# AnishDelft/ModelCompression

Measured on AMD Instinct MI355X. Metric: images/sec (fwd+bwd, 416x416), higher is better.
Workload: dtype fp16

## Files before the change

include/mcamd.h:

```cpp
#ifndef MCAMD_H
#define MCAMD_H

#include <stddef.h>
#include <stdint.h>

#ifdef __cplusplus
extern "C" {
#endif

#define MCAMD_OK 0
#define MCAMD_EINVAL (-1)
#define MCAMD_ELAUNCH (-2)
#define MCAMD_EWORKSPACE (-3)

int mcamd_version(void);
void mcamd_reload_config(void);
const char* mcamd_arch(void);
const char* mcamd_last_error(void);

typedef struct mcamd_conv_geom {
    int32_t B, H, W;
    int32_t ksize;
    int32_t cin;
    int32_t cout;
    int32_t x_ld;
    int32_t x_choff;
    int32_t stem;
    int32_t pad;
    int32_t x_wrap;
    int32_t x_f8;
    int32_t x_f8_wexp;
} mcamd_conv_geom;
int32_t mcamd_conv_fwd_f8_ok(const mcamd_conv_geom* g);

#define MCAMD_EPI_RAW_F16 0
#define MCAMD_EPI_NCHW_F32 1
#define MCAMD_EPI_PAD_F16 2
#define MCAMD_EPI_RAW_F32 3
typedef struct mcamd_conv_epilogue {
    int32_t mode;
    int32_t y_ld, y_choff;
    void* y;
    const float* bias;
    float* stats;
    int32_t stats_rows;
    int32_t stats_ld;
    const float* scale;
    const float* shift;
    float slope;
    int32_t* overflow;
    int32_t dst_mode;
    void* y2;
    int32_t y2_ld, y2_choff;
    int32_t concurrent;
} mcamd_conv_epilogue;

int32_t mcamd_conv_stats_rows(const mcamd_conv_geom* g);
int32_t mcamd_conv_stats_rows_mode(const mcamd_conv_geom* g, int32_t mode);

int mcamd_conv_tile_info(const mcamd_conv_geom* g, int32_t dgrad, int32_t out[4]);
int mcamd_conv_route_info(const mcamd_conv_geom* g, int32_t dir, int32_t mode, int32_t dst_mode, int32_t stats, int32_t out[5]);

int64_t mcamd_packed_elems_fwd(const mcamd_conv_geom* g);
int64_t mcamd_packed_elems_dgrad(const mcamd_conv_geom* g);

typedef struct mcamd_chan_map {
    const int32_t* rows;
    const int32_t* cols;
} mcamd_chan_map;

int mcamd_pack_weights(const mcamd_conv_geom* g, const float* w_oihw, const float* mask_oihw,
                       const mcamd_chan_map* map, void* wp_fwd, void* wp_dgrad, void* stream);

typedef struct mcamd_pack_job {
    const float* w;
    const float* mask;
    void* dst_fwd;
    void* dst_dgrad;
    const int32_t* rows;
    const int32_t* cols;
    int64_t first_tile;
    int32_t cout, cin, ksize;
    int32_t split;
    int32_t f8_wexp;
} mcamd_pack_job;
int mcamd_pack_weights_many(const mcamd_pack_job* jobs_dev, int32_t njobs, int64_t total_tiles, void* stream);

int mcamd_conv_fwd(const mcamd_conv_geom* g, const void* x, const void* wp_fwd,
                   const mcamd_conv_epilogue* epi, void* stream);

int32_t mcamd_conv_fwd_sparse24_ok(const mcamd_conv_geom* g);
int mcamd_sparse24_elems(const mcamd_conv_geom* g, int64_t out[2]);
int mcamd_conv_fwd_sparse24_info(const mcamd_conv_geom* g, int32_t out[7]);
int mcamd_pack_sparse24(const mcamd_conv_geom* g, const float* w_oihw, const float* mask_oihw, void* wsp, void* idx, void* stream);
int mcamd_conv_fwd_sparse24(const mcamd_conv_geom* g, const void* x, const void* wsp, const void* idx,
                            const mcamd_conv_epilogue* epi, void* stream);

int32_t mcamd_conv_fwd_bsparse_ok(const mcamd_conv_geom* g);
int mcamd_bsparse_elems(const mcamd_conv_geom* g, int64_t out[2]);
int mcamd_bsparse_lists(const mcamd_conv_geom* g, const void* wp_fwd, int32_t* count, int32_t* list, void* stream);
int mcamd_conv_fwd_bsparse(const mcamd_conv_geom* g, const void* x, const void* wp_fwd, const int32_t* count,
                           const int32_t* list, const mcamd_conv_epilogue* epi, void* stream);

typedef struct mcamd_splitk_info {
    int32_t slices;
    int32_t bm, bn, bk;
    int32_t chunks;
    int32_t tiles;
    int64_t workspace_bytes;
} mcamd_splitk_info;
int mcamd_conv_fwd_splitk_info(const mcamd_conv_geom* g, int32_t mode, int32_t dst_mode, int32_t slices,
                               mcamd_splitk_info* out);
int mcamd_conv_fwd_splitk(const mcamd_conv_geom* g, const void* x, const void* wp_fwd, const mcamd_conv_epilogue* epi,
                          int32_t slices, void* workspace, size_t workspace_bytes, void* stream);

int32_t mcamd_conv_fwd_q8_ok(const mcamd_conv_geom* g);
int mcamd_q8_elems(const mcamd_conv_geom* g, int64_t out[2]);
int mcamd_pack_q8(const mcamd_conv_geom* g, const float* w_oihw, const float* mask_oihw, void* wq, int32_t* wexp, void* stream);
int mcamd_conv_fwd_q8(const mcamd_conv_geom* g, const void* x8, const void* wq, const int32_t* wexp,
                      const mcamd_conv_epilogue* epi, int32_t y_f8, int32_t y2_f8, void* stream);
int mcamd_conv_fwd_q8_info(const mcamd_conv_geom* g, int32_t form, int32_t out[7]);
int mcamd_cast_q8(const void* src, int64_t pixels, int32_t src_ld, int32_t src_choff, int32_t C, void* dst, int32_t dst_ld,
                  int32_t dst_choff, void* stream);

int mcamd_conv_fwd_q8_splitk_info(const mcamd_conv_geom* g, int32_t dst_mode, int32_t slices, mcamd_splitk_info* out);
int mcamd_conv_fwd_q8_splitk(const mcamd_conv_geom* g, const void* x8, const void* wq, const int32_t* wexp,
                             const mcamd_conv_epilogue* epi, int32_t y_f8, int32_t y2_f8, int32_t slices, void* workspace,
                             size_t workspace_bytes, void* stream);

int32_t mcamd_conv_fwd_q8_slim_ok(const mcamd_conv_geom* g);
int mcamd_q8_slim_elems(const mcamd_conv_geom* g, int64_t out[2]);
int mcamd_pack_q8_slim(const mcamd_conv_geom* g, const float* w_oihw, const float* mask_oihw, void* wq, int32_t* wexp,
                       void* stream);
int mcamd_conv_fwd_q8_slim(const mcamd_conv_geom* g, const void* x8, const void* wq, const int32_t* wexp,
                           const mcamd_conv_epilogue* epi, const float* border, int32_t border_ld, int32_t y_f8, int32_t y2_f8,
                           void* stream);

int32_t mcamd_conv_fwd_q8_stats_rows(const mcamd_conv_geom* g);
int mcamd_fakequant_q8(const mcamd_conv_geom* g, const float* w_oihw, const float* mask_oihw, const int32_t* wexp,
                       float* wq_oihw, void* stream);
int mcamd_cast_q8_train(void* src, int64_t pixels, int32_t src_ld, int32_t src_choff, int32_t C, void* dst, int32_t dst_ld,
                        int32_t dst_choff, void* stream);

int32_t mcamd_conv_fwd_q8_sparse24_ok(const mcamd_conv_geom* g);
int mcamd_q8_sparse24_elems(const mcamd_conv_geom* g, int64_t out[3]);
int mcamd_pack_q8_sparse24(const mcamd_conv_geom* g, const float* w_oihw, const float* mask_oihw, void* wq, void* idx,
                           int32_t* wexp, void* stream);
int mcamd_conv_fwd_q8_sparse24(const mcamd_conv_geom* g, const void* x8, const void* wq, const void* idx, const int32_t* wexp,
                               const mcamd_conv_epilogue* epi, int32_t y_f8, int32_t y2_f8, void* stream);

int32_t mcamd_conv_fwd_q8_w4_ok(const mcamd_conv_geom* g);
int mcamd_q8_w4_elems(const mcamd_conv_geom* g, int64_t out[3]);
int mcamd_pack_q8_w4(const mcamd_conv_geom* g, const float* w_oihw, const float* mask_oihw, void* codes, void* gshift,
                     int32_t* wexp, void* stream);
int mcamd_unpack_q8_w4(const mcamd_conv_geom* g, const void* codes, const void* gshift, void* wq, void* stream);
int mcamd_conv_fwd_q8_w4(const mcamd_conv_geom* g, const void* x8, const void* codes, const void* gshift, const int32_t* wexp,
                         const mcamd_conv_epilogue* epi, int32_t y_f8, int32_t y2_f8, void* stream);
int mcamd_conv_fwd_q8_w4_info(const mcamd_conv_geom* g, int32_t out[7]);

int mcamd_conv_fwd_q8_w4_raw(const mcamd_conv_geom* g, const void* x8, const void* codes, const void* gshift, const int32_t* wexp,
                             const mcamd_conv_epilogue* epi, void* stream);
int mcamd_fakequant_q8_w4(const mcamd_conv_geom* g, const void* codes, const void* gshift, const int32_t* wexp, float* wq_oihw,
                          void* stream);

int mcamd_conv_dgrad(const mcamd_conv_geom* g, const void* dy, int32_t dy_ld, int32_t dy_choff,
                     const void* wp_dgrad, const mcamd_conv_epilogue* epi, void* stream);

typedef struct mcamd_dgrad_sums {
    float* slab;
    int32_t rows;
    int32_t ld;
    const void* act;
    int32_t act_ld, act_choff, act_pad;
    const float* scale; const float* shift; const float* mean; const float* invstd;
    float slope;
    const float* y;
    int32_t y_ld, y_choff;
    int32_t ch_lo, C;
} mcamd_dgrad_sums;
int32_t mcamd_conv_dgrad_sums_rows(const mcamd_conv_geom* g, int32_t concurrent);
int mcamd_conv_dgrad_sums(const mcamd_conv_geom* g, const void* dy, int32_t dy_ld, int32_t dy_choff,
                          const void* wp_dgrad, const mcamd_conv_epilogue* epi, const mcamd_dgrad_sums* sums, void* stream);

size_t mcamd_conv_wgrad_workspace_bytes(const mcamd_conv_geom* g);
int mcamd_conv_wgrad(const mcamd_conv_geom* g, const void* x, const void* dy, int32_t dy_ld,
                     int32_t dy_choff, const float* mask_oihw, const mcamd_chan_map* map,
                     float grad_scale, float* dw_oihw, float* dbias, void* workspace,
                     size_t workspace_bytes, void* stream);

#define MCAMD_WGRAD_GENERIC 0
#define MCAMD_WGRAD_STEM 1
#define MCAMD_WGRAD_WIN 2
#define MCAMD_WGRAD_NINE 3
#define MCAMD_WGRAD_NINE_WIDE 4
#define MCAMD_WFIN_ROW 0
#define MCAMD_WFIN_VEC 1
#define MCAMD_WFIN_GENERIC 2
#define MCAMD_WGRAD_PLAN_INFO_N 13
int mcamd_conv_wgrad_plan_info(const mcamd_conv_geom* g, int32_t has_cmap, int32_t out[MCAMD_WGRAD_PLAN_INFO_N]);
int32_t mcamd_wgrad_generic_instances(int32_t* out, int32_t cap);

int mcamd_bn_coeffs(const float* stats, int32_t stats_rows, int32_t stats_ld, int32_t C, int64_t count,
                    const float* gamma, const float* beta, float* running_mean, float* running_var,
                    float momentum, float eps, int32_t training,
                    float* scale, float* shift, float* save_mean, float* save_invstd,
                    const int32_t* chan_perm, void* stream);

int mcamd_bn_coeffs_ex(const float* stats, int32_t stats_rows, int32_t stats_ld, int32_t C, int64_t count,
                       const float* gamma, const float* beta, float* running_mean, float* running_var,
                       float momentum, float eps, int32_t training,
                       float* scale, float* shift, float* save_mean, float* save_invstd,
                       const int32_t* chan_perm, int32_t ones_channel, void* stream);

#define MCAMD_DST_PLAIN 0
// ... 296 lines not shown
```

modelcompression_amd/_lib.py:

```python
import ctypes as C
import os

_HERE = os.path.dirname(os.path.abspath(__file__))
LIB_PATH = os.path.join(_HERE, "libmcamd.so")


class McamdError(RuntimeError):
    pass


class ConvGeom(C.Structure):
    _fields_ = [("B", C.c_int32), ("H", C.c_int32), ("W", C.c_int32), ("ksize", C.c_int32),
                ("cin", C.c_int32), ("cout", C.c_int32), ("x_ld", C.c_int32), ("x_choff", C.c_int32),
                ("stem", C.c_int32), ("pad", C.c_int32), ("x_wrap", C.c_int32), ("x_f8", C.c_int32), ("x_f8_wexp", C.c_int32)]


class ConvEpilogue(C.Structure):
    _fields_ = [("mode", C.c_int32), ("y_ld", C.c_int32), ("y_choff", C.c_int32),
                ("y", C.c_void_p), ("bias", C.c_void_p), ("stats", C.c_void_p),
                ("stats_rows", C.c_int32), ("stats_ld", C.c_int32),
                ("scale", C.c_void_p), ("shift", C.c_void_p), ("slope", C.c_float), ("overflow", C.c_void_p),
                ("dst_mode", C.c_int32), ("y2", C.c_void_p), ("y2_ld", C.c_int32), ("y2_choff", C.c_int32),
                ("concurrent", C.c_int32)]

# ... 5 lines not shown
                ("dst", C.c_void_p), ("dst_ld", C.c_int32), ("dst_choff", C.c_int32),
                ("dst2", C.c_void_p), ("dst2_ld", C.c_int32), ("dst2_choff", C.c_int32),
                ("y_dtype", C.c_int32), ("planes", C.c_int32), ("dst_plane", C.c_int32), ("dst2_plane", C.c_int32),
                ("dst_pad", C.c_int32), ("dst2_pad", C.c_int32), ("border", C.c_void_p), ("planes2", C.c_int32),
                ("pool_act", C.c_void_p), ("pool_act_ld", C.c_int32), ("pool_act_pad", C.c_int32),
                ("dst_q8", C.c_void_p), ("dst2_q8", C.c_void_p)]


class ChanMap(C.Structure):
    _fields_ = [("rows", C.c_void_p), ("cols", C.c_void_p)]


class PackJob(C.Structure):
    _fields_ = [("w", C.c_void_p), ("mask", C.c_void_p), ("dst_fwd", C.c_void_p), ("dst_dgrad", C.c_void_p),
                ("rows", C.c_void_p), ("cols", C.c_void_p),
                ("first_tile", C.c_int64), ("cout", C.c_int32), ("cin", C.c_int32), ("ksize", C.c_int32),
                ("split", C.c_int32), ("f8_wexp", C.c_int32)]


class ActBwdDesc(C.Structure):
    _fields_ = [("B", C.c_int32), ("H", C.c_int32), ("W", C.c_int32), ("C", C.c_int32),
                ("y", C.c_void_p), ("y_ld", C.c_int32), ("y_choff", C.c_int32),
                ("scale", C.c_void_p), ("shift", C.c_void_p), ("mean", C.c_void_p), ("invstd", C.c_void_p),
                ("slope", C.c_float), ("mode", C.c_int32),
                ("g", C.c_void_p), ("g_ld", C.c_int32), ("g_choff", C.c_int32),
                ("g2", C.c_void_p), ("g2_ld", C.c_int32), ("g2_choff", C.c_int32),
                ("dy", C.c_void_p), ("dy_ld", C.c_int32), ("dy_choff", C.c_int32),
                ("dgamma", C.c_void_p), ("dbeta", C.c_void_p), ("grad_scale", C.c_float),
                ("dy_keep", C.c_void_p), ("chan_perm", C.c_void_p), ("y_dtype", C.c_int32),
                ("overflow", C.c_void_p), ("dy_pad", C.c_int32), ("skip_dead_param_grads", C.c_int32),
                ("act", C.c_void_p), ("act_ld", C.c_int32), ("act_choff", C.c_int32), ("act_pad", C.c_int32),
                ("pool_out", C.c_void_p), ("pool_out_ld", C.c_int32), ("pool_out_choff", C.c_int32),
                ("pool_out_pad", C.c_int32),
                ("sums", C.c_void_p), ("sums_rows", C.c_int32), ("sums_ld", C.c_int32)]


class DgradSums(C.Structure):
    _fields_ = [("slab", C.c_void_p), ("rows", C.c_int32), ("ld", C.c_int32),
                ("act", C.c_void_p), ("act_ld", C.c_int32), ("act_choff", C.c_int32), ("act_pad", C.c_int32),
                ("scale", C.c_void_p), ("shift", C.c_void_p), ("mean", C.c_void_p), ("invstd", C.c_void_p),
                ("slope", C.c_float), ("y", C.c_void_p), ("y_ld", C.c_int32), ("y_choff", C.c_int32),
                ("ch_lo", C.c_int32), ("C", C.c_int32)]


class SplitkInfo(C.Structure):
    _fields_ = [("slices", C.c_int32), ("bm", C.c_int32), ("bn", C.c_int32), ("bk", C.c_int32),
                ("chunks", C.c_int32), ("tiles", C.c_int32), ("workspace_bytes", C.c_int64)]


class FoldDesc(C.Structure):
    _fields_ = [("w", C.c_void_p), ("mask", C.c_void_p), ("rows", C.c_void_p), ("cols", C.c_void_p),
                ("beta", C.c_void_p), ("slope", C.c_float),
                ("n", C.c_int32), ("cin_t", C.c_int32), ("cin_k", C.c_int32), ("cin_aug", C.c_int32), ("ksize", C.c_int32)]


class StemBlockDesc(C.Structure):
    _fields_ = [("B", C.c_int32), ("H", C.c_int32), ("W", C.c_int32),
                ("x", C.c_void_p), ("wp", C.c_void_p), ("gamma", C.c_void_p), ("beta", C.c_void_p),
                ("running_mean", C.c_void_p), ("running_var", C.c_void_p),
                ("momentum", C.c_float), ("eps", C.c_float), ("training", C.c_int32),
                ("scale", C.c_void_p), ("shift", C.c_void_p), ("save_mean", C.c_void_p), ("save_invstd", C.c_void_p),
                ("slope", C.c_float),
                ("dst", C.c_void_p), ("dst_ld", C.c_int32), ("dst_choff", C.c_int32),
                ("g", C.c_void_p), ("g_ld", C.c_int32), ("g_choff", C.c_int32),
                ("mask", C.c_void_p), ("grad_scale", C.c_float),
                ("dw", C.c_void_p), ("dgamma", C.c_void_p), ("dbeta", C.c_void_p), ("cout", C.c_int32), ("planes", C.c_int32),
                ("x_lo", C.c_void_p), ("wp_lo", C.c_void_p)]


class RegionDesc(C.Structure):
    _fields_ = [("output", C.c_void_p), ("target", C.c_void_p),
                ("B", C.c_int32), ("H", C.c_int32), ("W", C.c_int32), ("num_anchors", C.c_int32), ("num_classes", C.c_int32),
                ("max_boxes", C.c_int32), ("anchors", C.c_float * 16),
                ("coord_scale", C.c_float), ("noobject_scale", C.c_float), ("object_scale", C.c_float),
                ("class_scale", C.c_float), ("thresh", C.c_float)]


class DistillDesc(C.Structure):
    _fields_ = [("student", C.c_void_p), ("teacher", C.c_void_p),
                ("B", C.c_int32), ("H", C.c_int32), ("W", C.c_int32), ("num_anchors", C.c_int32), ("num_classes", C.c_int32),
                ("obj_scale", C.c_float), ("box_scale", C.c_float), ("cls_scale", C.c_float), ("temperature", C.c_float)]


class DetectDesc(C.Structure):
    _fields_ = [("output", C.c_void_p),
                ("B", C.c_int32), ("H", C.c_int32), ("W", C.c_int32), ("num_anchors", C.c_int32), ("num_classes", C.c_int32),
                ("anchors", C.c_float * 16), ("conf_thresh", C.c_float), ("nms_thresh", C.c_float)]


class VocMatchDesc(C.Structure):
    _fields_ = [("rows", C.c_void_p), ("probs", C.c_void_p), ("nkept", C.c_void_p),
                ("B", C.c_int32), ("N", C.c_int32), ("C", C.c_int32), ("G", C.c_int32),
                ("conf_thresh", C.c_float), ("first_image", C.c_int32), ("ovthresh", C.c_double),
                ("gt_box", C.c_void_p), ("gt_cls", C.c_void_p), ("gt_difficult", C.c_void_p), ("gt_count", C.c_void_p),
                ("image_size", C.c_void_p),
                ("keys", C.c_void_p), ("flags", C.c_void_p), ("capacity", C.c_int64), ("counters", C.c_void_p)]


class FoldJob(C.Structure):
    _fields_ = [("d", FoldDesc), ("waug", C.c_void_p), ("first_block", C.c_int64)]


class AugmentDesc(C.Structure):
    _fields_ = [("src_off", C.c_int64), ("tmp_off", C.c_int64),
                ("src_w", C.c_int32), ("src_h", C.c_int32), ("crop_x", C.c_int32), ("crop_y", C.c_int32),
                ("crop_w", C.c_int32), ("crop_h", C.c_int32), ("flip", C.c_int32),
                ("hk", C.c_int32), ("vk", C.c_int32), ("hcoef_off", C.c_int32), ("vcoef_off", C.c_int32),
                ("lut_off", C.c_int32)]


class AugmentBatch(C.Structure):
    _fields_ = [("desc", C.c_void_p), ("desc_dev", C.c_void_p),
                ("src", C.c_void_p), ("src_bytes", C.c_int64),
                ("coef", C.c_void_p), ("coef_elems", C.c_int64),
                ("lut", C.c_void_p), ("lut_bytes", C.c_int64),
                ("tmp", C.c_void_p), ("tmp_bytes", C.c_int64),
                ("out", C.c_void_p), ("B", C.c_int32), ("H", C.c_int32), ("W", C.c_int32)]


class WzSeg(C.Structure):
    _fields_ = [("w", C.c_void_p), ("mask", C.c_void_p), ("n", C.c_int64), ("word0", C.c_int64), ("val0", C.c_int64),
                ("kept", C.c_int64), ("cout", C.c_int32), ("kind", C.c_int32), ("exp0", C.c_int32), ("dense", C.c_int32),
                ("block0", C.c_int32), ("reserved", C.c_int32)]


class WsSeg(C.Structure):
    _fields_ = [("w", C.c_void_p), ("mask", C.c_void_p), ("codes", C.c_void_p), ("n", C.c_int64), ("part0", C.c_int64),
                ("K", C.c_int32), ("cb0", C.c_int32), ("slab0", C.c_int32), ("reserved", C.c_int32)]


EPI_RAW_F16, EPI_NCHW_F32, EPI_PAD_F16, EPI_RAW_F32 = 0, 1, 2, 3
DST_PLAIN, DST_POOL, DST_REORG = 0, 1, 2
WGRAD_GENERIC, WGRAD_STEM, WGRAD_WIN, WGRAD_NINE, WGRAD_NINE_WIDE = 0, 1, 2, 3, 4
WFIN_ROW, WFIN_VEC, WFIN_GENERIC = 0, 1, 2
WGRAD_PLAN_INFO_N = 13
STEM_PLAN_FWD, STEM_PLAN_FWD_PLANES, STEM_PLAN_STATS, STEM_PLAN_GRAM, STEM_PLAN_BWD = 0, 1, 2, 3, 4
STEM_PLAN_INFO_N = 20
WZ_FP32, WZ_FP16, WZ_FP8, WZ_CODE = 0, 1, 2, 4
WZ_F_BN, WZ_F_BITS = 1, 2
WZ_BLOCK_WORDS = 64
WS_SLAB = 4096

_P, _I32, _I64, _F, _SZ = C.c_void_p, C.c_int32, C.c_int64, C.c_float, C.c_size_t
SIGNATURES = {
    "mcamd_version": (C.c_int, []),
    "mcamd_arch": (C.c_char_p, []),
    "mcamd_last_error": (C.c_char_p, []),
    "mcamd_reload_config": (None, []),
    "mcamd_conv_stats_rows": (_I32, [C.POINTER(ConvGeom)]),
    "mcamd_conv_stats_rows_mode": (_I32, [C.POINTER(ConvGeom), _I32]),
    "mcamd_conv_fwd_f8_ok": (_I32, [C.POINTER(ConvGeom)]),
    "mcamd_conv_tile_info": (C.c_int, [C.POINTER(ConvGeom), _I32, C.POINTER(_I32)]),
    "mcamd_conv_route_info": (C.c_int, [C.POINTER(ConvGeom), _I32, _I32, _I32, _I32, C.POINTER(_I32)]),
    "mcamd_packed_elems_fwd": (_I64, [C.POINTER(ConvGeom)]),
    "mcamd_packed_elems_dgrad": (_I64, [C.POINTER(ConvGeom)]),
    "mcamd_pack_weights": (C.c_int, [C.POINTER(ConvGeom), _P, _P, C.POINTER(ChanMap), _P, _P, _P]),
    "mcamd_pack_weights_many": (C.c_int, [_P, _I32, _I64, _P]),
    "mcamd_conv_fwd": (C.c_int, [C.POINTER(ConvGeom), _P, _P, C.POINTER(ConvEpilogue), _P]),
    "mcamd_conv_fwd_sparse24_ok": (_I32, [C.POINTER(ConvGeom)]),
    "mcamd_sparse24_elems": (C.c_int, [C.POINTER(ConvGeom), C.POINTER(_I64)]),
    "mcamd_conv_fwd_sparse24_info": (C.c_int, [C.POINTER(ConvGeom), C.POINTER(_I32)]),
    "mcamd_pack_sparse24": (C.c_int, [C.POINTER(ConvGeom), _P, _P, _P, _P, _P]),
    "mcamd_conv_fwd_sparse24": (C.c_int, [C.POINTER(ConvGeom), _P, _P, _P, C.POINTER(ConvEpilogue), _P]),
    "mcamd_conv_fwd_bsparse_ok": (_I32, [C.POINTER(ConvGeom)]),
    "mcamd_bsparse_elems": (C.c_int, [C.POINTER(ConvGeom), C.POINTER(_I64)]),
    "mcamd_bsparse_lists": (C.c_int, [C.POINTER(ConvGeom), _P, _P, _P, _P]),
    "mcamd_conv_fwd_bsparse": (C.c_int, [C.POINTER(ConvGeom), _P, _P, _P, _P, C.POINTER(ConvEpilogue), _P]),
    "mcamd_conv_fwd_splitk_info": (C.c_int, [C.POINTER(ConvGeom), _I32, _I32, _I32, C.POINTER(SplitkInfo)]),
    "mcamd_conv_fwd_splitk": (C.c_int, [C.POINTER(ConvGeom), _P, _P, C.POINTER(ConvEpilogue), _I32, _P, _SZ, _P]),
    "mcamd_conv_fwd_q8_ok": (_I32, [C.POINTER(ConvGeom)]),
    "mcamd_q8_elems": (C.c_int, [C.POINTER(ConvGeom), C.POINTER(_I64)]),
    "mcamd_pack_q8": (C.c_int, [C.POINTER(ConvGeom), _P, _P, _P, _P, _P]),
    "mcamd_conv_fwd_q8": (C.c_int, [C.POINTER(ConvGeom), _P, _P, _P, C.POINTER(ConvEpilogue), _I32, _I32, _P]),
    "mcamd_conv_fwd_q8_info": (C.c_int, [C.POINTER(ConvGeom), _I32, C.POINTER(_I32)]),
    "mcamd_conv_fwd_q8_splitk_info": (C.c_int, [C.POINTER(ConvGeom), _I32, _I32, C.POINTER(SplitkInfo)]),
    "mcamd_conv_fwd_q8_splitk": (C.c_int, [C.POINTER(ConvGeom), _P, _P, _P, C.POINTER(ConvEpilogue), _I32, _I32, _I32, _P, _SZ, _P]),
    "mcamd_conv_fwd_q8_slim_ok": (_I32, [C.POINTER(ConvGeom)]),
    "mcamd_q8_slim_elems": (C.c_int, [C.POINTER(ConvGeom), C.POINTER(_I64)]),
    "mcamd_pack_q8_slim": (C.c_int, [C.POINTER(ConvGeom), _P, _P, _P, _P, _P]),
    "mcamd_conv_fwd_q8_slim": (C.c_int, [C.POINTER(ConvGeom), _P, _P, _P, C.POINTER(ConvEpilogue), _P, _I32, _I32, _I32, _P]),
    "mcamd_conv_fwd_q8_sparse24_ok": (_I32, [C.POINTER(ConvGeom)]),
    "mcamd_q8_sparse24_elems": (C.c_int, [C.POINTER(ConvGeom), C.POINTER(_I64)]),
    "mcamd_pack_q8_sparse24": (C.c_int, [C.POINTER(ConvGeom), _P, _P, _P, _P, _P, _P]),
    "mcamd_conv_fwd_q8_sparse24": (C.c_int, [C.POINTER(ConvGeom), _P, _P, _P, _P, C.POINTER(ConvEpilogue), _I32, _I32, _P]),
    "mcamd_conv_fwd_q8_w4_ok": (_I32, [C.POINTER(ConvGeom)]),
    "mcamd_q8_w4_elems": (C.c_int, [C.POINTER(ConvGeom), C.POINTER(_I64)]),
    "mcamd_pack_q8_w4": (C.c_int, [C.POINTER(ConvGeom), _P, _P, _P, _P, _P, _P]),
    "mcamd_unpack_q8_w4": (C.c_int, [C.POINTER(ConvGeom), _P, _P, _P, _P]),
    "mcamd_conv_fwd_q8_w4": (C.c_int, [C.POINTER(ConvGeom), _P, _P, _P, _P, C.POINTER(ConvEpilogue), _I32, _I32, _P]),
    "mcamd_conv_fwd_q8_w4_info": (C.c_int, [C.POINTER(ConvGeom), C.POINTER(_I32)]),
    "mcamd_conv_fwd_q8_w4_raw": (C.c_int, [C.POINTER(ConvGeom), _P, _P, _P, _P, C.POINTER(ConvEpilogue), _P]),
    "mcamd_fakequant_q8_w4": (C.c_int, [C.POINTER(ConvGeom), _P, _P, _P, _P, _P]),
    "mcamd_cast_q8": (C.c_int, [_P, _I64, _I32, _I32, _I32, _P, _I32, _I32, _P]),
    "mcamd_conv_fwd_q8_stats_rows": (_I32, [C.POINTER(ConvGeom)]),
    "mcamd_fakequant_q8": (C.c_int, [C.POINTER(ConvGeom), _P, _P, _P, _P, _P]),
    "mcamd_cast_q8_train": (C.c_int, [_P, _I64, _I32, _I32, _I32, _P, _I32, _I32, _P]),
    "mcamd_conv_dgrad": (C.c_int, [C.POINTER(ConvGeom), _P, _I32, _I32, _P, C.POINTER(ConvEpilogue), _P]),
    "mcamd_conv_dgrad_sums_rows": (_I32, [C.POINTER(ConvGeom), _I32]),
    "mcamd_conv_dgrad_sums": (C.c_int, [C.POINTER(ConvGeom), _P, _I32, _I32, _P, C.POINTER(ConvEpilogue), C.POINTER(DgradSums), _P]),
    "mcamd_conv_wgrad_workspace_bytes": (_SZ, [C.POINTER(ConvGeom)]),
    "mcamd_conv_wgrad": (C.c_int, [C.POINTER(ConvGeom), _P, _P, _I32, _I32, _P, C.POINTER(ChanMap), _F, _P, _P, _P, _SZ, _P]),
    "mcamd_conv_wgrad_plan_info": (C.c_int, [C.POINTER(ConvGeom), _I32, C.POINTER(_I32)]),
    "mcamd_wgrad_generic_instances": (_I32, [C.POINTER(_I32), _I32]),
    "mcamd_bn_coeffs": (C.c_int, [_P, _I32, _I32, _I32, _I64, _P, _P, _P, _P, _F, _F, _I32, _P, _P, _P, _P, _P, _P]),
    "mcamd_bn_coeffs_ex": (C.c_int, [_P, _I32, _I32, _I32, _I64, _P, _P, _P, _P, _F, _F, _I32, _P, _P, _P, _P, _P, _I32, _P]),
    "mcamd_fold_weights": (C.c_int, [C.POINTER(FoldDesc), _P, _P]),
    "mcamd_fold_weights_many": (C.c_int, [_P, _I32, _I64, _P]),
    "mcamd_unfold_wgrad": (C.c_int, [C.POINTER(FoldDesc), _P, _P, _P, _P, _I32, _P]),
    "mcamd_bn_act_fwd": (C.c_int, [C.POINTER(ActDesc), _P]),
    "mcamd_bn_act_conv1x1_ok": (_I32, [C.POINTER(ActDesc), C.POINTER(ConvGeom)]),
    "mcamd_bn_act_conv1x1_stats_rows": (_I32, [C.POINTER(ActDesc), C.POINTER(ConvGeom)]),
    "mcamd_bn_act_conv1x1_fwd": (C.c_int, [C.POINTER(ActDesc), C.POINTER(ConvGeom), _P, C.POINTER(ConvEpilogue), _P]),
    "mcamd_bn_act_bwd_workspace_bytes": (_SZ, [C.POINTER(ActBwdDesc)]),
    "mcamd_bn_act_bwd": (C.c_int, [C.POINTER(ActBwdDesc), _P, _SZ, _P]),
    "mcamd_stem_block_workspace_bytes": (_SZ, []),
    "mcamd_stem_block_fwd": (C.c_int, [C.POINTER(StemBlockDesc), _P, _SZ, _P]),
    "mcamd_stem_block_bwd": (C.c_int, [C.POINTER(StemBlockDesc), _P, _SZ, _P]),
    "mcamd_stem_block_stats_rows": (_I32, [C.POINTER(StemBlockDesc)]),
    "mcamd_stem_block_stats": (C.c_int, [C.POINTER(StemBlockDesc), _P, _I32, _I32, _P]),
    "mcamd_stem_block_plan_info": (C.c_int, [C.POINTER(StemBlockDesc), C.POINTER(_I32)]),
    "mcamd_nchw_f32_to_nhwc4_split": (C.c_int, [_P, _I32, _I32, _I32, _P, _P, _P]),
    "mcamd_pack_stem_split": (C.c_int, [_P, _P, _I32, _P, _P, _P]),
    "mcamd_nchw_f32_to_padded_nhwc_f16": (C.c_int, [_P, _I32, _I32, _I32, _I32, _F, _P, _I32, _I32, _P, _P]),
    "mcamd_nchw_f32_to_padded_nhwc_f16_pad": (C.c_int, [_P, _I32, _I32, _I32, _I32, _F, _P, _I32, _I32, _I32, _P, _P]),
    "mcamd_nchw_f32_to_padded_nhwc_f16_split": (C.c_int, [_P, _I32, _I32, _I32, _I32, _P, _I32, _I32, _I32, _P]),
    "mcamd_stem_conv_f32_stats_rows": (_I32, []),
    "mcamd_stem_conv_f32": (C.c_int, [_P, _I32, _I32, _I32, _P, _P, _I32, _P, _P, _I32, _P, _I32, _I32, _P]),
    "mcamd_region_loss_workspace_bytes": (_SZ, [_I32]),
    "mcamd_region_loss": (C.c_int, [C.POINTER(RegionDesc), _P, _P, _P, _P, _SZ, _P]),
    "mcamd_distill_loss_workspace_bytes": (_SZ, [_I32, _I32]),
    "mcamd_distill_loss": (C.c_int, [C.POINTER(DistillDesc), _P, _P, _P, _SZ, _P]),
    "mcamd_region_decode": (C.c_int, [C.POINTER(DetectDesc), _P, _P, _P]),
    "mcamd_nms": (C.c_int, [_P, _P, _I32, _I32, _F, _P, _P, _P]),
    "mcamd_detect": (C.c_int, [C.POINTER(DetectDesc), _P, _P, _P, _P, _P, _P]),
    "mcamd_voc_match": (C.c_int, [C.POINTER(VocMatchDesc), _P]),
    "mcamd_voc_ap": (C.c_int, [_P, _P, _P, _I64, _P, _I32, _P, _P, _P, _P]),
    "mcamd_augment": (C.c_int, [C.POINTER(AugmentBatch), _P]),
    "mcamd_augment_tables": (C.c_int, [_P, _P, _P, _I32, _I32, _I32, _P, _I64, _P, _I64, _P]),
    "mcamd_plan_begin": (C.c_int, [C.POINTER(_P), _I32]),
    "mcamd_plan_mark": (_I32, []),
    "mcamd_plan_end": (_P, []),
    "mcamd_plan_segments": (_I32, [_P]),
    "mcamd_plan_launches": (_I32, [_P]),
    "mcamd_plan_run": (C.c_int, [_P, _I32, _I32, C.POINTER(_P), _I32]),
    "mcamd_plan_destroy": (None, [_P]),
    "mcamd_stream_wait": (C.c_int, [_P, _P]),
    "mcamd_memset_zero": (C.c_int, [_P, _SZ, _P]),
    "mcamd_step_flags": (C.c_int, [_P, _I32, _P, _P, _P, _P, _P]),
    "mcamd_kth_magnitude_workspace_bytes": (_SZ, []),
    "mcamd_kth_magnitude": (C.c_int, [C.POINTER(_P), C.POINTER(_I64), _I32, _I64, _P, _P, _SZ, _P]),
    "mcamd_magnitude_mask": (C.c_int, [_P, _I64, _P, _P, _P]),
    "mcamd_filter_scores_workspace_bytes": (_SZ, [_I32]),
    "mcamd_filter_scores": (C.c_int, [_P, _I32, _I32, _I32, _I32, _P, _P, _SZ, _P]),
    "mcamd_filter_mean_square": (C.c_int, [_P, _I32, _I32, _I32, _I32, _P, _P, _SZ, _P]),
    "mcamd_filter_mask": (C.c_int, [_P, _I32, _I64, _P, _P]),
    "mcamd_count_zeros": (C.c_int, [_P, _I64, _P, _P]),
    "mcamd_masked_residual": (C.c_int, [_P, _P, _I64, _P, _P]),
    "mcamd_nm_mask": (C.c_int, [_P, _P, _I32, _I32, _I32, _I32, _I32, _P, _P]),
    "mcamd_nm_violations": (C.c_int, [_P, _I32, _I32, _I32, _P, _P]),
    "mcamd_block_scores": (C.c_int, [_P, _P, _I32, _I32, _I32, _P, _P]),
    "mcamd_block_mask": (C.c_int, [_P, _P, _I32, _I32, _I32, _P, _P]),
    "mcamd_wz_workspace_bytes": (_SZ, [_I64, _I32]),
    "mcamd_wz_pack": (C.c_int, [_P, _P, _I32, _P, _I64, _P, _P, _I64, _P, _I64, _P, _SZ, _P]),
    "mcamd_wz_unpack": (C.c_int, [_P, _P, _I32, _P, _I64, _P, _I64, _P, _I64, _P, _SZ, _P]),
    "mcamd_ws_workspace_bytes": (_SZ, [_I64, _I64, _I32]),
    "mcamd_ws_init": (C.c_int, [_P, _P, _I32, _P, _I64, _P, _SZ, _P]),
    "mcamd_ws_iterate": (C.c_int, [_P, _P, _I32, _P, _I64, _P, _P, _P, _SZ, _P]),
    "mcamd_ws_assign": (C.c_int, [_P, _P, _I32, _P, _I64, _P]),
    "mcamd_ws_project": (C.c_int, [_P, _P, _I32, _P, _I64, _P, _P, _P, _SZ, _P]),
    "mcamd_ws_expand": (C.c_int, [_P, _P, _I32, _P, _I64, _P]),
}

_lib = None


def lib():
    global _lib
    if _lib is None:
        if not os.path.exists(LIB_PATH):
            raise McamdError(
                "libmcamd.so is missing (%s). Build it with `python -m modelcompression_amd.build`; "
                "modelcompression_amd has no CPU/PyTorch fallback for its compute path." % LIB_PATH)
        import torch
        h = C.CDLL(LIB_PATH)
        for name, (res, args) in SIGNATURES.items():
            fn = getattr(h, name)
            fn.restype = res
            fn.argtypes = args
        _lib = h
    return _lib


def reload_config():
    lib().mcamd_reload_config()


def check(rc, what=""):
    if rc != 0:
        msg = lib().mcamd_last_error().decode()
        raise McamdError("%s failed (%d): %s" % (what or "mcamd call", rc, msg))


def ptr(t):
    return None if t is None else C.c_void_p(t.data_ptr())


# ... 4 lines not shown
```

modelcompression_amd/csrc/conv_small.hip:

```cpp
#include "kernels.h"
#include <stdlib.h>

template <int CT, int NB, int U>
__global__ __launch_bounds__(256, 1) void small3x3_kernel(IgemmArgs a) {
    constexpr int KK = CT / 32;
    constexpr int NC = NB * 16;
    constexpr int RC = NC / 8;
    static_assert(9 * KK * NB <= 36, "weights must fit 144 registers");
    static_assert(64 % RC == 0, "a lane must keep its channel piece across store passes");
    const int tid = threadIdx.x, lane = tid & 63, wave = tid >> 6;
    const int pl = lane & 15, kg = lane >> 4;

    h8_t wf[9][KK][NB];
#pragma unroll
    for (int t = 0; t < 9; ++t)
#pragma unroll
        for (int kk = 0; kk < KK; ++kk)
#pragma unroll
            for (int nb = 0; nb < NB; ++nb)
                wf[t][kk][nb] = *(const h8_t*)(a.w + (long long)(nb * 16 + pl) * a.ktot + t * CT + 32 * kk + 8 * kg);

    float s1[8], s2[8];
#pragma unroll
    for (int e = 0; e < 8; ++e) s1[e] = s2[e] = 0.f;
// ... 59 lines not shown
            const int piece = pass * 64 + lane;
            const int prow = piece / RC, pc = piece - prow * RC;
            if (U * 16 * RC % 64 != 0 && piece >= U * 16 * RC) break;
            const h8_t v = *(const h8_t*)(tw + prow * NC + pc * 8);
            if (m0 + prow < a.M && pc * 8 < a.N) {
                *(h8_t*)(y + (m0 + prow) * a.y_ld + a.y_choff + pc * 8) = v;
                if (want_stats) {
#pragma unroll
                    for (int e = 0; e < 8; ++e) {
                        const float f = (float)v[e];
                        s1[e] += f;
                        s2[e] += f * f;
                    }
                }
            }
        }
    }

    if (want_stats) {
        __shared__ float red[4][2][NC];
#pragma unroll
        for (int e = 0; e < 8; ++e) {
            float v1 = s1[e], v2 = s2[e];
#pragma unroll
            for (int msk = RC; msk < 64; msk <<= 1) {
                v1 += __shfl_xor(v1, msk);
                v2 += __shfl_xor(v2, msk);
            }
            if (lane < RC) {
                red[wave][0][lane * 8 + e] = v1;
                red[wave][1][lane * 8 + e] = v2;
            }
        }
        __syncthreads();
        for (int t = tid; t < 2 * NC; t += 256) {
            const int which = t / NC, n = t - which * NC;
            a.stats[((long long)blockIdx.x * 2 + which) * a.stats_ld + n] =
                red[0][which][n] + red[1][which][n] + red[2][which][n] + red[3][which][n];
        }
    }
}

template <int NB>
__global__ __launch_bounds__(256, 1) void small3x3_split_kernel(IgemmArgs a) {
    constexpr int NC = NB * 16;
    constexpr int RC = NC / 4;
    static_assert(64 % RC == 0, "a lane must keep its channel piece across store passes");
    const int tid = threadIdx.x, lane = tid & 63, wave = tid >> 6;
    const int pl = lane & 15, kg = lane >> 4;

    h8_t wh[9][NB], wl[9][NB];
#pragma unroll
    for (int t = 0; t < 9; ++t)
#pragma unroll
        for (int nb = 0; nb < NB; ++nb) {
            const half_t* wrow = a.w + (long long)(nb * 16 + pl) * a.ktot + t * 32 + 8 * kg;
            wh[t][nb] = *(const h8_t*)wrow;
            wl[t][nb] = *(const h8_t*)(wrow + 2 * 9 * 32);
        }

    float s1[4], s2[4];
#pragma unroll
    for (int e = 0; e < 4; ++e) s1[e] = s2[e] = 0.f;

    __shared__ __attribute__((aligned(16))) float tile[4][16 * NC];
    float* tw = tile[wave];
    const bool want_stats = a.stats != nullptr;

    const long long nunits = ((long long)a.M + 15) / 16;
    const long long per_wg = (nunits + gridDim.x - 1) / gridDim.x;
    const long long u_begin = (long long)blockIdx.x * per_wg;
    const long long u_end = u_begin + per_wg < nunits ? u_begin + per_wg : nunits;

    auto pix_ptr = [&](long long unit) {
        const long long m = unit * 16 + pl;
        const long long mc = m < a.M ? m : a.M - 1;
        const int b = (int)(mc / a.HW);
        const int rem = (int)(mc - (long long)b * a.HW);
        const int h = rem / a.W, w = rem - h * a.W;
        return a.x + (long long)b * a.x_img_stride + (long long)h * a.x_row_stride + (long long)w * a.x_ld + a.x_off + 8 * kg;
    };
    h8_t xh[9], xl[9];
    if (u_begin + wave < u_end) {
        const half_t* px = pix_ptr(u_begin + wave);
#pragma unroll
        for (int t = 0; t < 9; ++t) {
            xh[t] = *(const h8_t*)(px + a.tap_off[t]);
            xl[t] = *(const h8_t*)(px + a.tap_off[t] + 32);
        }
    }
    for (long long unit = u_begin + wave; unit < u_end; unit += 4) {
        const long long nxt = unit + 4 < u_end ? unit + 4 : unit;
        const half_t* pn = pix_ptr(nxt);
        f32x4_t acc[NB];
#pragma unroll
        for (int nb = 0; nb < NB; ++nb) acc[nb] = f32x4_t{0.f, 0.f, 0.f, 0.f};
#pragma unroll
        for (int t = 0; t < 9; ++t) {
#pragma unroll
            for (int nb = 0; nb < NB; ++nb) {
                acc[nb] = __builtin_amdgcn_mfma_f32_16x16x32_f16(wh[t][nb], xl[t], acc[nb], 0, 0, 0);
                acc[nb] = __builtin_amdgcn_mfma_f32_16x16x32_f16(wl[t][nb], xh[t], acc[nb], 0, 0, 0);
                acc[nb] = __builtin_amdgcn_mfma_f32_16x16x32_f16(wh[t][nb], xh[t], acc[nb], 0, 0, 0);
            }
            xh[t] = *(const h8_t*)(pn + a.tap_off[t]);
            xl[t] = *(const h8_t*)(pn + a.tap_off[t] + 32);
        }
#pragma unroll
        for (int nb = 0; nb < NB; ++nb) *(f32x4_t*)(tw + pl * NC + nb * 16 + 4 * kg) = acc[nb];
        const long long m0 = unit * 16;
        float* y = (float*)a.y;
#pragma unroll
        for (int pass = 0; pass < 16 * RC / 64; ++pass) {
            const int piece = pass * 64 + lane;
            const int prow = piece / RC, pc = piece - prow * RC;
            const f32x4_t v = *(const f32x4_t*)(tw + prow * NC + pc * 4);
            if (m0 + prow < a.M && pc * 4 < a.N) {
                *(f32x4_t*)(y + (m0 + prow) * a.y_ld + a.y_choff + pc * 4) = v;
                if (want_stats) {
#pragma unroll
                    for (int e = 0; e < 4; ++e) {
                        s1[e] += v[e];
                        s2[e] = __builtin_fmaf(v[e], v[e], s2[e]);
                    }
                }
            }
        }
    }

    if (want_stats) {
        __shared__ float red[4][2][NC];
#pragma unroll
        for (int e = 0; e < 4; ++e) {
            float v1 = s1[e], v2 = s2[e];
#pragma unroll
            for (int msk = RC; msk < 64; msk <<= 1) {
                v1 += __shfl_xor(v1, msk);
                v2 += __shfl_xor(v2, msk);
            }
            if (lane < RC) {
                red[wave][0][lane * 4 + e] = v1;
                red[wave][1][lane * 4 + e] = v2;
            }
        }
        __syncthreads();
        for (int t = tid; t < 2 * NC; t += 256) {
            const int which = t / NC, n = t - which * NC;
            a.stats[((long long)blockIdx.x * 2 + which) * a.stats_ld + n] =
                red[0][which][n] + red[1][which][n] + red[2][which][n] + red[3][which][n];
        }
    }
}

bool mcamd_small3x3_split_ok(long long M, int n, int cin_tap, int ktot, int wrap, int mode) {
    if (MCAMD_ENV_INT("MCAMD_SMALL3X3", 1) == 0) return false;
    return mode == MCAMD_EPI_RAW_F32 && cin_tap == 96 && ktot == 9 * 96 && wrap == 64 && n % 8 == 0 && n > 32 && n <= 64 &&
           M >= 4096;
}

int mcamd_small3x3_split_launch(const IgemmArgs& a, int grid, hipStream_t st) {
    hipLaunchKernelGGL((small3x3_split_kernel<4>), dim3(grid), dim3(256), 0, st, a);
    MCAMD_LAUNCH_CHECK("small3x3_split");
    return MCAMD_OK;
}


static int small_blocks(int n) { return n <= 16 ? 1 : n <= 32 ? 2 : 4; }

bool mcamd_small3x3_ok(long long M, int n, int cin_tap, int ktot) {
    const int lvl = MCAMD_ENV_INT("MCAMD_SMALL3X3", 1);
    if (lvl == 0) return false;
    if (ktot != 9 * cin_tap || n % 8 != 0 || n > 64 || M < 4096) return false;
    if (cin_tap == 32) return true;
    return lvl >= 2 && cin_tap == 64 && n <= 32;
}

int mcamd_small3x3_rows(long long M) {
    long long units = (M + 31) / 32, wgs = (units + 7) / 8;
    return (int)(wgs < 256 ? wgs : 256);
}

template <int CT, int NB>
static void launch_small(const IgemmArgs& a, int grid, hipStream_t st) {
    hipLaunchKernelGGL((small3x3_kernel<CT, NB, 2>), dim3(grid), dim3(256), 0, st, a);
}

int mcamd_small3x3_launch(const IgemmArgs& a, int grid, hipStream_t st) {
    const int nb = small_blocks(a.N);
    if (a.cin_tap == 32) {
        if (nb == 1) launch_small<32, 1>(a, grid, st);
        else if (nb == 2) launch_small<32, 2>(a, grid, st);
        else launch_small<32, 4>(a, grid, st);
    } else {
        if (nb == 1) launch_small<64, 1>(a, grid, st);
        else launch_small<64, 2>(a, grid, st);
    }
    MCAMD_LAUNCH_CHECK("small3x3");
    return MCAMD_OK;
}
```

Before: 5644.

## Add sliding-window row-ring variant of split small 3x3 conv kernel

Adds a new split small-3x3 kernel that walks image row segments per wave. Input rows are staged asynchronously into a seven-slot LDS ring, so each row loaded is reused across the three vertical taps. Output tile stores are interleaved between MFMA taps to overlap writes with compute. The launcher picks a segment height from a cost model and defaults to the new path when W/H/M shapes qualify. A launch counter is exported for inspection, and the change adds heavy LDS use and complex vmcnt bookkeeping.

After: 5690 (median of 6 runs). Within noise of the previous version (+0.8%).

```diff
diff --git a/include/mcamd.h b/include/mcamd.h
--- a/include/mcamd.h
+++ b/include/mcamd.h
@@ -60,6 +60,7 @@
 
 int mcamd_conv_tile_info(const mcamd_conv_geom* g, int32_t dgrad, int32_t out[4]);
 int mcamd_conv_route_info(const mcamd_conv_geom* g, int32_t dir, int32_t mode, int32_t dst_mode, int32_t stats, int32_t out[5]);
+int64_t mcamd_small3x3_split_launches(int32_t form);
 
 int64_t mcamd_packed_elems_fwd(const mcamd_conv_geom* g);
 int64_t mcamd_packed_elems_dgrad(const mcamd_conv_geom* g);
diff --git a/modelcompression_amd/_lib.py b/modelcompression_amd/_lib.py
--- a/modelcompression_amd/_lib.py
+++ b/modelcompression_amd/_lib.py
@@ -181,6 +181,7 @@
     "mcamd_conv_fwd_f8_ok": (_I32, [C.POINTER(ConvGeom)]),
     "mcamd_conv_tile_info": (C.c_int, [C.POINTER(ConvGeom), _I32, C.POINTER(_I32)]),
     "mcamd_conv_route_info": (C.c_int, [C.POINTER(ConvGeom), _I32, _I32, _I32, _I32, C.POINTER(_I32)]),
+    "mcamd_small3x3_split_launches": (_I64, [_I32]),
     "mcamd_packed_elems_fwd": (_I64, [C.POINTER(ConvGeom)]),
     "mcamd_packed_elems_dgrad": (_I64, [C.POINTER(ConvGeom)]),
     "mcamd_pack_weights": (C.c_int, [C.POINTER(ConvGeom), _P, _P, C.POINTER(ChanMap), _P, _P, _P]),
diff --git a/modelcompression_amd/csrc/conv_small.hip b/modelcompression_amd/csrc/conv_small.hip
--- a/modelcompression_amd/csrc/conv_small.hip
+++ b/modelcompression_amd/csrc/conv_small.hip
@@ -235,15 +235,301 @@
     }
 }
 
+namespace {
+constexpr int WN_NR = 7;
+constexpr int WN_ROW_BYTES = 5 * 1024;
+constexpr int WN_LA = 3;
+constexpr int WN_TILE_BYTES = 16 * 68 * 4;
+constexpr int WN_WAVE_BYTES = WN_NR * WN_ROW_BYTES + WN_TILE_BYTES;
+constexpr int WN_MAX_STORES = 32;
+}
+
+template <int LO, int HI>
+__device__ __forceinline__ void split_win_wait_sel(int stores) {
+    if constexpr (LO == HI) {
+        wait_vmcnt<5 * WN_LA + LO>();
+    } else {
+        constexpr int MID = (LO + HI) / 2;
+        if (stores <= MID) split_win_wait_sel<LO, MID>(stores);
+        else split_win_wait_sel<MID + 1, HI>(stores);
+    }
+}
+__device__ __forceinline__ void split_win_wait(int stores) {
+    static_assert(5 * WN_LA + WN_MAX_STORES <= 63, "vmcnt is a 6-bit counter");
+    split_win_wait_sel<0, WN_MAX_STORES>(stores < WN_MAX_STORES ? stores : WN_MAX_STORES);
+}
+
+template <int NB>
+__global__ __launch_bounds__(256, 1) void small3x3_split_win_kernel(IgemmArgs a, int nseg, int nstrips) {
+    constexpr int NC = NB * 16;
+    constexpr int RC = NC / 4;
+    constexpr int PPP = 64 / RC;
+    static_assert(64 % RC == 0, "a lane must keep its channel piece across store passes");
+    constexpr int TLD = NC + 4;
+    static_assert(16 * TLD * 4 <= WN_TILE_BYTES, "the wave's output tile");
+    extern __shared__ __attribute__((aligned(16))) char smem[];
+    const int tid = threadIdx.x, lane = tid & 63;
+    const int wave = __builtin_amdgcn_readfirstlane(tid >> 6);
+    char* ring = smem + wave * WN_WAVE_BYTES;
+    float* tw = (float*)(ring + WN_NR * WN_ROW_BYTES);
+    const int pl = lane & 15, kg = lane >> 4;
+
+    h8_t wh[9][NB], wl[9][NB];
+#pragma unroll
+    for (int t = 0; t < 9; ++t)
+#pragma unroll
+        for (int nb = 0; nb < NB; ++nb) {
+            const half_t* wrow = a.w + (long long)(nb * 16 + pl) * a.ktot + t * 32 + 8 * kg;
+            wh[t][nb] = *(const h8_t*)wrow;
+            wl[t][nb] = *(const h8_t*)(wrow + 2 * 9 * 32);
+        }
+
+    float s1[4], s2[4];
+#pragma unroll
+    for (int e = 0; e < 4; ++e) s1[e] = s2[e] = 0.f;
+    const bool want_stats = a.stats != nullptr;
+
+    unsigned src_off[5];
+#pragma unroll
+    for (int it = 0; it < 5; ++it) {
+        int q = it * 64 + lane;
+        if (q > 271) q = 271;
+        const int P = q >> 3;
+        src_off[it] = (unsigned)(P * a.x_ld + (((q & 7) ^ (((P >> 1) & 3) << 1)) * 8));
+    }
+    auto stage_row = [&](const half_t* rowp, int slot) {
+        char* dst = ring + slot * WN_ROW_BYTES;
+#pragma unroll
+        for (int it = 0; it < 5; ++it) glds16(rowp + src_off[it], dst + it * 1024);
+    };
+    int off_h[3];
+#pragma unroll
+    for (int tx = 0; tx < 3; ++tx) {
+        const int P = pl + tx;
+        off_h[tx] = P * 128 + ((kg ^ (((P >> 1) & 3) << 1)) * 16);
+    }
+
+    const int lane_row = lane / RC, lane_pc = lane - lane_row * RC;
+    const unsigned lane_yoff = (unsigned)(lane_row * a.y_ld + lane_pc * 4);
+
+    struct Unit {
+        const half_t* xs;
+        float* y0;
+        int nrows, ng;
+        int w_left;
+        bool ok;
+    };
+    const int nunits = a.M / (a.H * a.W) * nstrips * nseg;
+    const int nwaves = gridDim.x * 4, gw = blockIdx.x * 4 + wave;
+    auto unit_of = [&](int u) {
+        Unit q;
+        q.ok = u < nunits;
+        if (!q.ok) u = nunits - 1;
+        const int seg = u % nseg, rest = u / nseg;
+        const int strip = rest % nstrips, b = rest / nstrips;
+        const int h_lo = (int)((long long)seg * a.H / nseg), h_hi = (int)((long long)(seg + 1) * a.H / nseg);
+        const int c0 = strip * 32;
+        q.nrows = h_hi - h_lo;
+        q.w_left = a.W - c0;
+        q.ng = q.w_left > 16 ? 2 : 1;
+        q.xs = a.x + (long long)b * a.x_img_stride + (long long)h_lo * a.x_row_stride + (long long)c0 * a.x_ld + a.x_off;
+        q.y0 = (float*)a.y + ((long long)(b * a.H + h_lo) * a.W + c0) * a.y_ld + a.y_choff;
+        return q;
+    };
+
+    int st_issued = 0, st_m0 = 0, st_m1 = 0, st_m2 = 0, st_m3 = 0;
+    int slot_in = 0;
+    int unit_slot0 = 0, pre = 0;
+    float* pend_yg = (float*)a.y;
+    int pend_valid = 0;
+    f32x4_t pv;
+    auto pass_read = [&](int pass) { pv = *(const f32x4_t*)(tw + (pass * PPP + lane_row) * TLD + lane_pc * 4); };
+    auto pass_store = [&](int pass) {
+        if (lane_row < pend_valid - pass * PPP && lane_pc * 4 < a.N) {
+            *(f32x4_t*)(pend_yg + (long long)(pass * PPP) * a.y_ld + lane_yoff) = pv;
+            if (want_stats) {
+#pragma unroll
+                for (int e = 0; e < 4; ++e) {
+                    s1[e] += pv[e];
+                    s2[e] = __builtin_fmaf(pv[e], pv[e], s2[e]);
+                }
+            }
+        }
+        st_issued += pass * PPP < pend_valid ? 1 : 0;
+    };
+
+    Unit nxt = unit_of(gw);
+    for (int unit = gw; unit < nunits; unit += nwaves) {
+        const Unit cur = nxt;
+        nxt = unit_of(unit + nwaves);
+        int own_next = pre, nxt_staged = 0;
+        auto stage_one = [&]() {
+            const half_t* rowp;
+            if (own_next <= cur.nrows + 1) rowp = cur.xs + (long long)own_next++ * a.x_row_stride;
+            else if (nxt.ok) {
+                const int r = nxt_staged < nxt.nrows + 1 ? nxt_staged : nxt.nrows + 1;
+                rowp = nxt.xs + (long long)r * a.x_row_stride;
+                ++nxt_staged;
+            } else rowp = cur.xs + (long long)(cur.nrows + 1) * a.x_row_stride;
+            stage_row(rowp, slot_in);
+            slot_in = slot_in + 1 == WN_NR ? 0 : slot_in + 1;
+            st_m3 = st_m2, st_m2 = st_m1, st_m1 = st_m0, st_m0 = st_issued;
+        };
+        for (int r = pre; r < 2 + WN_LA; ++r) stage_one();
+        const int ng = cur.ng, nrows = cur.nrows;
+        const int ngroups_unit = nrows * ng;
+        int rk = 0, rgi = 0, slot0 = unit_slot0;
+        const char *r0, *r1, *r2;
+        auto begin_row = [&]() {
+            stage_one();
+            split_win_wait(st_issued - st_m3);
+            int sl1 = slot0 + 1, sl2 = slot0 + 2;
+            if (sl1 >= WN_NR) sl1 -= WN_NR;
+            if (sl2 >= WN_NR) sl2 -= WN_NR;
+            r0 = ring + slot0 * WN_ROW_BYTES;
+            r1 = ring + sl1 * WN_ROW_BYTES;
+            r2 = ring + sl2 * WN_ROW_BYTES;
+            slot0 = slot0 + 1 == WN_NR ? 0 : slot0 + 1;
+        };
+        auto read_group = [&](h8_t (&xh)[9], h8_t (&xl)[9]) {
+#pragma unroll
+            for (int t = 0; t < 9; ++t) {
+                const char* rp = (t / 3 == 0 ? r0 : t / 3 == 1 ? r1 : r2) + rgi * (16 * 128);
+                xh[t] = *(const h8_t*)(rp + off_h[t % 3]);
+                xl[t] = *(const h8_t*)(rp + (off_h[t % 3] ^ 64));
+            }
+        };
+        auto fetch_next = [&](h8_t (&xh)[9], h8_t (&xl)[9]) {
+            if (++rgi == ng) {
+                rgi = 0;
+                if (++rk < nrows) begin_row();
+            }
+            if (rk < nrows) read_group(xh, xl);
+        };
+        int cgi = 0;
+        float* yrow = cur.y0;
+        auto compute = [&](const h8_t (&xh)[9], const h8_t (&xl)[9]) {
+            f32x4_t acc[NB];
+#pragma unroll
+            for (int nb = 0; nb < NB; ++nb) acc[nb] = f32x4_t{0.f, 0.f, 0.f, 0.f};
+#pragma unroll
+            for (int t = 0; t < 9; ++t) {
+#pragma unroll
+                for (int nb = 0; nb < NB; ++nb) {
+                    acc[nb] = __builtin_amdgcn_mfma_f32_16x16x32_f16(wh[t][nb], xl[t], acc[nb], 0, 0, 0);
+                    acc[nb] = __builtin_amdgcn_mfma_f32_16x16x32_f16(wl[t][nb], xh[t], acc[nb], 0, 0, 0);
+                    acc[nb] = __builtin_amdgcn_mfma_f32_16x16x32_f16(wh[t][nb], xh[t], acc[nb], 0, 0, 0);
+                }
+                static_assert(16 * RC / 64 == 4, "four store passes between nine taps");
+                if (t < 8) {
+                    __builtin_amdgcn_sched_barrier(0);
+                    if (t % 2 == 0) pass_read(t / 2);
+                    else pass_store(t / 2);
+                    __builtin_amdgcn_sched_barrier(0);
+                }
+            }
+            __builtin_amdgcn_s_waitcnt(0xC07F);
+#pragma unroll
+            for (int nb = 0; nb < NB; ++nb) *(f32x4_t*)(tw + pl * TLD + nb * 16 + 4 * kg) = acc[nb];
+            const int valid = cur.w_left - cgi * 16;
+            pend_valid = valid < 16 ? valid : 16;
+            pend_yg = yrow + (long long)(cgi * 16) * a.y_ld;
+            if (++cgi == ng) {
+                cgi = 0;
+                yrow += (long long)a.W * a.y_ld;
+            }
+        };
+
+        h8_t xh0[9], xl0[9], xh1[9], xl1[9];
+        begin_row();
+        read_group(xh0, xl0);
+        __builtin_amdgcn_s_waitcnt(0xC07F);
+        for (int j = 0; j < ngroups_unit; j += 2) {
+            __builtin_amdgcn_sched_barrier(0);
+            fetch_next(xh1, xl1);
+            __builtin_amdgcn_sched_barrier(0);
+            compute(xh0, xl0);
+            if (j + 1 < ngroups_unit) {
+                __builtin_amdgcn_sched_barrier(0);
+                fetch_next(xh0, xl0);
+                __builtin_amdgcn_sched_barrier(0);
+                compute(xh1, xl1);
+            }
+        }
+        pre = nxt_staged;
+        unit_slot0 = (unit_slot0 + nrows + 2) % WN_NR;
+    }
+#pragma unroll
+    for (int pass = 0; pass < 16 * RC / 64; ++pass) {
+        pass_read(pass);
+        pass_store(pass);
+    }
+
+    if (want_stats) {
+        __shared__ float red[4][2][NC];
+#pragma unroll
+        for (int e = 0; e < 4; ++e) {
+            float v1 = s1[e], v2 = s2[e];
+#pragma unroll
+            for (int msk = RC; msk < 64; msk <<= 1) {
+                v1 += __shfl_xor(v1, msk);
+                v2 += __shfl_xor(v2, msk);
+            }
+            if (lane < RC) {
+                red[wave][0][lane * 4 + e] = v1;
+                red[wave][1][lane * 4 + e] = v2;
+            }
+        }
+        __syncthreads();
+        for (int t = tid; t < 2 * NC; t += 256) {
+            const int which = t / NC, n = t - which * NC;
+            a.stats[((long long)blockIdx.x * 2 + which) * a.stats_ld + n] =
+                red[0][which][n] + red[1][which][n] + red[2][which][n] + red[3][which][n];
+        }
+    }
+}
+
 bool mcamd_small3x3_split_ok(long long M, int n, int cin_tap, int ktot, int wrap, int mode) {
     if (MCAMD_ENV_INT("MCAMD_SMALL3X3", 1) == 0) return false;
     return mode == MCAMD_EPI_RAW_F32 && cin_tap == 96 && ktot == 9 * 96 && wrap == 64 && n % 8 == 0 && n > 32 && n <= 64 &&
            M >= 4096;
 }
 
+static int split_form(const IgemmArgs& a) {
+    if (MCAMD_ENV_INT("MCAMD_SMALL3X3_SPLIT_WIN", 1) == 0) return 0;
+    return a.W >= 16 && a.W % 2 == 0 && a.H >= 4 && a.M % ((long long)a.H * a.W) == 0 ? 1 : 0;
+}
+
+static long long g_split_launches[2];
+
+extern "C" int64_t mcamd_small3x3_split_launches(int32_t form) {
+    return form == 0 || form == 1 ? __atomic_load_n(&g_split_launches[form], __ATOMIC_RELAXED) : -1;
+}
+
 int mcamd_small3x3_split_launch(const IgemmArgs& a, int grid, hipStream_t st) {
-    hipLaunchKernelGGL((small3x3_split_kernel<4>), dim3(grid), dim3(256), 0, st, a);
-    MCAMD_LAUNCH_CHECK("small3x3_split");
+    const int form = split_form(a);
+    if (form == 0) {
+        hipLaunchKernelGGL((small3x3_split_kernel<4>), dim3(grid), dim3(256), 0, st, a);
+        MCAMD_LAUNCH_CHECK("small3x3_split");
+    } else {
+        const int nstrips = (a.W + 31) / 32;
+        const long long runners = (long long)grid * 4;
+        const long long per_row_units = (long long)(a.M / ((long long)a.H * a.W)) * nstrips;
+        int want = 8;
+        double best = 1e30;
+        for (int sg = 8; sg <= 32; ++sg) {
+            const int ns = (a.H + sg - 1) / sg, rows = (a.H + ns - 1) / ns;
+            const long long rounds = (per_row_units * ns + runners - 1) / runners;
+            const double cost = (double)rounds * (rows + 2);
+            if (cost < best - 1e-9) best = cost, want = sg;
+        }
+        const int nseg = (a.H + want - 1) / want;
+        const size_t lds = 4 * (size_t)WN_WAVE_BYTES;
+        MCAMD_LDS_OPT_IN((small3x3_split_win_kernel<4>), lds);
+        hipLaunchKernelGGL((small3x3_split_win_kernel<4>), dim3(grid), dim3(256), lds, st, a, nseg, nstrips);
+        MCAMD_LAUNCH_CHECK("small3x3_split_win");
+    }
+    __atomic_add_fetch(&g_split_launches[form], 1, __ATOMIC_RELAXED);
     return MCAMD_OK;
 }
 
```
